# BowieHsu/tensorflow_ocr

Measured on AMD Instinct MI355X. Metric: images/sec training, 512x512 ICDAR, VGG-16 EAST, batch 32, 1/2/4/8 GPU, higher is better.
Workload: dtype f16; 1 GPU; VGG-16 model_vgg + dice loss train step, 512x512, batch 32 per GPU, f16 storage / f32 accumulate, Adam+EMA; global_batch=32, parallelism=dp1

## Files before the change

include/ocr_hip.h:

```cpp
#ifndef OCR_HIP_H_
#define OCR_HIP_H_

#include <stddef.h>
#include <stdint.h>

#ifdef __cplusplus
extern "C" {
#endif

#define OCR_ABI_VERSION 7

enum {
  OCR_OK = 0,
  OCR_ERR_INVALID_ARG = -1,
  OCR_ERR_UNSUPPORTED = -2,
  OCR_ERR_HIP = -3,
  OCR_ERR_WORKSPACE = -4,
  OCR_ERR_RCCL = -5
};

int ocr_abi_version(void);
const char* ocr_status_string(int status);
const char* ocr_storage_dtype(void);
uint32_t ocr_crc32c(const void* data, size_t n, uint32_t seed);
// ... 96 lines not shown
                        const void* bias, int flags, void* y, void* stats, void* stream);
size_t ocr_conv2d_stem_wgrad_workspace(int n, int h, int w, int cout);
int ocr_conv2d_stem_wgrad_f16(int n, int h, int w, int cout, const void* x4, const void* dy,
                              void* dw_hwio_f32, void* workspace, size_t ws_bytes, void* stream);
int ocr_conv2d_stem_wgrad_bn_f16(int n, int h, int w, int cout, const void* x4, const void* da, const void* bn_y,
                                 const void* bn_shift, const void* coef_a, const void* coef_b, const void* coef_c,
                                 int relu, void* dw, void* workspace, size_t ws_bytes, void* stream);
int ocr_pack_weights_f16(const void* w_hwio_f32, int taps, int cin, int cout, void* w_kc,
                         void* w_ck, void* stream);
int ocr_pack_weights_first_f16(const void* w_hwio_f32, int cout, void* w_first, void* stream);
size_t ocr_conv2d_first_moments_workspace(void);
int ocr_conv2d_first_moments_f16(int n, int h, int w, int cout, const void* x4, const void* w_first, void* stats_row,
                                 void* workspace, size_t ws_bytes, void* stream);
int ocr_conv2d_first_moments_keep_f16(int n, int h, int w, int cout, const void* x4, const void* w_first,
                                      void* stats_row, void* moments_f64, void* workspace, size_t ws_bytes, void* stream);
size_t ocr_pack_weights_batch_table_bytes(int n);
int ocr_pack_weights_batch_table(int n, const void* const* w_hwio_f32, const int* taps, const int* cin,
                                 const int* cout, void* const* w_kc, void* const* w_ck, const int* ld_ck,
                                 void* table_host, int* grid_out);
int ocr_pack_weights_batch_f16(const void* table_dev, int n, int grid, void* stream);
int ocr_pack_weights_small_f16(const void* w_f32, int cin, int cout, void* w_kc32, void* w_ck32,
                               void* stream);

int ocr_prep_images_f16(const void* images_f32, int64_t npix, float m0, float m1, float m2,
                        void* out_f16x4, void* stream);
int ocr_prep_images_norm_f16(const void* images_f32, int64_t npix, float m0, float m1, float m2,
                             float div, void* out_f16x4, void* stream);

size_t ocr_bn_reduce_workspace(int T, int C);
int ocr_bn_finalize(const void* partial, int T, int C, double count, const void* gamma,
// ... 448 lines not shown
```

tensorflow_ocr_amd/csrc/bn_pool.hip:

```cpp
#include "common.h"
#include "pool_gather.h"

namespace {

__global__ void prep_images_kernel(const float* __restrict__ img, half_t* __restrict__ out,
                                   size_t npix, float m0, float m1, float m2, float div) {
  size_t i = (size_t)blockIdx.x * blockDim.x + threadIdx.x;
  if (i >= npix) return;
  float r = (img[i * 3 + 0] - m0) / div, g = (img[i * 3 + 1] - m1) / div, b = (img[i * 3 + 2] - m2) / div;
  half4_t o = {(half_t)r, (half_t)g, (half_t)b, (half_t)0.f};
  *reinterpret_cast<half4_t*>(out + i * 4) = o;
}

struct BnFin {
  double count;
  const float *gamma, *beta;
  float eps, decay;
  float *moving_mean, *moving_var, *scale, *shift, *save_mean, *save_invstd;
};
struct BnBwdFin {
  float *dgamma, *dbeta;
};
struct BnBwdFinC {
  float *dgamma, *dbeta;
  const float *scale, *mean, *invstd;
  float inv_count;
  float *A, *B, *C;
};

constexpr int kTicketGroup = 32, kTicketGroups = 128;
__device__ unsigned ocr_bn_tickets[16 * 32 * (1 + kTicketGroups)];

template <typename FIN>
__device__ __forceinline__ void bn_fin_apply(const FIN& f, int c, double s, double q);

template <>
__device__ __forceinline__ void bn_fin_apply<BnFin>(const BnFin& f, int c, double s, double q) {
  double mean = s / f.count;
  double var = q / f.count - mean * mean;
  if (var < 0.0) var = 0.0;
  float invstd = (float)(1.0 / sqrt(var + (double)f.eps));
  float g = f.gamma ? f.gamma[c] : 1.f;
  float b = f.beta ? f.beta[c] : 0.f;
  float sc = g * invstd;
  f.scale[c] = sc;
  f.shift[c] = b - (float)mean * sc;
  if (f.save_mean) f.save_mean[c] = (float)mean;
  if (f.save_invstd) f.save_invstd[c] = invstd;
  if (f.moving_mean) {
    double unbiased = f.count > 1.0 ? var * f.count / (f.count - 1.0) : var;
    f.moving_mean[c] = f.moving_mean[c] * f.decay + (float)mean * (1.f - f.decay);
    f.moving_var[c] = f.moving_var[c] * f.decay + (float)unbiased * (1.f - f.decay);
  }
}

template <>
__device__ __forceinline__ void bn_fin_apply<BnBwdFin>(const BnBwdFin& f, int c, double s, double q) {
  f.dbeta[c] = (float)s;
  f.dgamma[c] = (float)q;
}

template <>
__device__ __forceinline__ void bn_fin_apply<BnBwdFinC>(const BnBwdFinC& f, int c, double s, double q) {
  f.dbeta[c] = (float)s;
  f.dgamma[c] = (float)q;
  const float sc = f.scale[c], mu = f.mean[c], is = f.invstd[c];
  const float k_dz = (float)s * f.inv_count, k_dzx = (float)q * f.inv_count;
  f.A[c] = sc;
  f.B[c] = -sc * is * k_dzx;
  f.C[c] = sc * (mu * is * k_dzx - k_dz);
}

static inline int red_rows(int T) {
  if (T <= 1024) return (T + 63) / 64 * 64;
  int rows = ((T + 15) / 16 + 31) / 32 * 32;
  if (rows < 256) rows = 256;
  if (rows > 2048) rows = 2048;
  return rows;
}

template <typename FIN>
__global__ __launch_bounds__(256) void reduce_finalize_kernel(const float* __restrict__ partial,
                                                              double* __restrict__ stage, int T, int C, int slot,
                                                              int rows, FIN fin) {
  __shared__ double red[16][2][64];
  __shared__ unsigned s_ticket;
  const int cl = threadIdx.x & 15, rl = threadIdx.x >> 4;
  const int c4 = blockIdx.y * 64 + cl * 4;
  const int t0 = blockIdx.x * rows;
  const int R = gridDim.x;
  double s[4] = {0.0, 0.0, 0.0, 0.0}, q[4] = {0.0, 0.0, 0.0, 0.0};
  const bool live = c4 < C;
  const bool vec = (C & 3) == 0;
  if (live) {
// ... 1489 lines not shown
```

tensorflow_ocr_amd/csrc/conv_first.hip:

```cpp
#include "common.h"
#include "conv_epilogue.h"

namespace {

constexpr int HW = 36;

struct FirstP {
  int n, h, w, cout, tiles_x, tiles_y, m_tiles, flags;
};

__device__ __forceinline__ void load_halo4(const half_t* __restrict__ x4, char* halo, int img, int h,
                                           int w, int iy0, int ix0) {
  for (int i = threadIdx.x; i < 10 * HW; i += 256) {
    const int hy = i / HW, hx = i - hy * HW;
    const int iy = iy0 + hy, ix = ix0 + hx;
    u32x2 v = {0u, 0u};
    if (iy >= 0 && iy < h && ix >= 0 && ix < w)
      v = *reinterpret_cast<const u32x2*>(x4 + (((size_t)img * h + iy) * w + ix) * 4);
    *reinterpret_cast<u32x2*>(halo + i * 8) = v;
  }
}

__device__ __forceinline__ void first_weights(const half_t* __restrict__ wf, int cout, int co0, int lane,
                                              half8_t (&a)[3][2]) {
// ... 365 lines not shown
        s2 += wv[i] * t;
      }
    }
    part[0][rl][threadIdx.x & 63] = s1;
    part[1][rl][threadIdx.x & 63] = s2;
    __syncthreads();
    if (threadIdx.x < 128) {
      const int k = threadIdx.x >> 6, cc = threadIdx.x & 63;
      if (c0 + cc < cout)
        row[k * cout + c0 + cc] = (float)(((part[k][0][cc] + part[k][1][cc]) + part[k][2][cc]) + part[k][3][cc]);
    }
    __syncthreads();
  }
}

__global__ __launch_bounds__(256) void first_wgrad_sums_kernel(const float* __restrict__ s1, int blocks,
                                                               const double* __restrict__ M,
                                                               const half_t* __restrict__ wf,
                                                               const float* __restrict__ A, const float* __restrict__ B,
                                                               const float* __restrict__ C, float* __restrict__ dw) {
  __shared__ double red[2][4][64];
  __shared__ double Mrow[32];
  const int k = blockIdx.x;
  const int ky = k / 9, kx = (k / 3) % 3, ch = k % 3;
  const int slot = ky * 10 + kx * 3 + ch;
  const int c = threadIdx.x & 63, bl = threadIdx.x >> 6;
  if (threadIdx.x < 32) Mrow[threadIdx.x] = M[k * 32 + threadIdx.x];
  float wj[7];
#pragma unroll
  for (int u = 0; u < 7; ++u) {
// ... 13 lines not shown
    for (int u = 0; u < 16; ++u) acc += (double)v[u];
  }
  __syncthreads();
  double mw = 0.0;
#pragma unroll
  for (int u = 0; u < 7; ++u) {
    const int j = bl + 4 * u;
    if (j < 27) mw += Mrow[j] * (double)wj[u];
  }
  red[0][bl][c] = acc;
  red[1][bl][c] = mw;
  __syncthreads();
  if (threadIdx.x < 64) {
    const double S1 = (red[0][0][c] + red[0][1][c]) + (red[0][2][c] + red[0][3][c]);
    const double MW = (red[1][0][c] + red[1][1][c]) + (red[1][2][c] + red[1][3][c]);
    dw[k * 64 + c] = (float)((double)A[c] * S1 + (double)B[c] * MW + (double)C[c] * M[27 * 32 + k]);
  }
}

__global__ void first_reduce_kernel(const float* __restrict__ partial, float* __restrict__ dw,
                                    int elems, int blocks) {
  int i = blockIdx.x * blockDim.x + threadIdx.x;
  if (i >= elems) return;
  float a = 0.f;
  for (int b = 0; b < blocks; ++b) a += partial[(size_t)b * elems + i];
  dw[i] = a;
}

__global__ void pack_first_kernel(const float* __restrict__ w, half_t* __restrict__ out, int cout) {
  int i = blockIdx.x * blockDim.x + threadIdx.x;
  if (i >= 3 * cout * 16) return;
// ... 142 lines not shown
                     cout, static_cast<float*>(stats_row), static_cast<double*>(moments_f64));
  return ocr_launch_status();
}

extern "C" int ocr_conv2d_first_wgrad_sums_f32(const void* s1_blocks, int blocks, const void* moments_f64,
                                               const void* w_first, int cout, const void* coef_a, const void* coef_b,
                                               const void* coef_c, void* dw, void* stream) {
  OCR_CHECK_ARG(s1_blocks && blocks > 0 && moments_f64 && w_first && coef_a && coef_b && coef_c && dw);
  OCR_CHECK_SHAPE(cout == 64);
  hipLaunchKernelGGL(first_wgrad_sums_kernel, dim3(27), dim3(256), 0, static_cast<hipStream_t>(stream),
                     static_cast<const float*>(s1_blocks), blocks, static_cast<const double*>(moments_f64),
                     static_cast<const half_t*>(w_first), static_cast<const float*>(coef_a),
                     static_cast<const float*>(coef_b), static_cast<const float*>(coef_c), static_cast<float*>(dw));
  return ocr_launch_status();
}
```

tensorflow_ocr_amd/graph.py:

```python
import contextlib
import math

import numpy as np
import torch

from . import _lib as L
from . import ops

F16, F32 = (torch.bfloat16 if L.STORAGE == "bf16" else torch.float16), torch.float32


class Variable:

    def __init__(self, name, shape, init, trainable, regularized):
        self.name = name
        self.shape = tuple(int(s) for s in shape)
        self.init = init
        self.trainable = trainable
        self.regularized = regularized
        self.data = None
        self.grad = None
        self.packed = {}

    @property
# ... 96 lines not shown
        for n, arr in sd.items():
            if n not in self.vars:
                if strict:
                    raise KeyError(n)
                continue
            v = self.vars[n]
            a = np.asarray(arr, dtype=np.float32).reshape(v.shape)
            v.data.copy_(torch.from_numpy(a))
        self.version += 1


class Act:

    __slots__ = ("_data", "grad", "requires_grad", "name", "bn_ctx", "bn_partial", "tail_ctx", "tail_partial",
                 "pending", "sub_grad", "deferred", "tail_fwd", "pending_owner", "consumed", "bn_fwd", "bias_ctx",
                 "bias_partial", "sole_consumer", "bias_done", "pool_grad", "takes_pool_grad", "first_s1")

    def __init__(self, data, requires_grad=True, name=""):
        self._data = data
        self.grad = None
        self.requires_grad = requires_grad
        self.name = name
        self.bn_ctx = None
        self.bn_partial = None
        self.tail_ctx = None
        self.tail_partial = None
        self.pending = None
        self.pending_owner = None
        self.consumed = False
        self.sub_grad = None
        self.deferred = None
        self.bias_ctx = None
        self.bias_partial = None
        self.bias_done = False
        self.sole_consumer = False
        self.takes_pool_grad = False
        self.pool_grad = None
        self.first_s1 = None
        self.bn_fwd = None
        self.tail_fwd = None

    @property
    def data(self):
        if self.deferred is not None:
            fill, self.deferred = self.deferred, None
            fill()
        return self._data

    @data.setter
    def data(self, value):
        self._data = value

    @property
# ... 281 lines not shown
```

tensorflow_ocr_amd/layers.py:

```python
import torch

from . import ops
from .graph import Act, F16, F32, constant, variance_scaling, xavier_uniform
from ._lib import CONV_ACCUM_F16, CONV_BIAS, CONV_RELU, CONV_STATS

BN_DECAY = 0.997
BN_EPS = 1e-5
FUSE_BN_REDUCE = __import__("os").environ.get("OCR_FUSE_BN", "1") == "1"


def _bn_vars(g, C):
    with g.variable_scope("BatchNorm"):
        gamma = g.get_variable("gamma", (C,), constant(1.0))
        beta = g.get_variable("beta", (C,), constant(0.0))
        mm = g.get_variable("moving_mean", (C,), constant(0.0), trainable=False)
        mv = g.get_variable("moving_variance", (C,), constant(1.0), trainable=False)
    return gamma, beta, mm, mv


def _packs(g, w, first):
    kh, kw, cin, cout = w.shape
    if first:
        def mk(old):
            t = old if old is not None else g.empty((3, cout, 16))
            ops.pack_weights_first(w.data, t)
            return t
        return g.packed(w, "first", mk), None

    def mk(old):
        if old is None:
            old = (g.empty((kh * kw, cout, cin)), g.empty((kh * kw, cin, cout)))
        ops.pack_weights(w.data, old[0], old[1])
        return old
    return g.packed(w, "kc_ck", mk)


FUSE_BIAS_POOL = __import__("os").environ.get("OCR_FUSE_BIAS_POOL", "1") == "1"
FUSE_BIAS_RELU = __import__("os").environ.get("OCR_FUSE_BIAS_RELU", "1") == "1"


# ... 2 lines not shown
    t = cache.get((n, value))
    if t is None:
        t = cache[(n, value)] = torch.full((n,), float(value), dtype=F32, device=g.device)
    return t


FUSE_BN_W4_MAXHW = int(__import__("os").environ.get("OCR_FUSE_BN_W4_MAXHW", "1000000"))
FUSE_BN_POOL_REDUCE = __import__("os").environ.get("OCR_FUSE_BN_POOL_REDUCE", "1") == "1"
FIRST_RECOMPUTE = __import__("os").environ.get("OCR_FIRST_RECOMPUTE", "1") == "1"
FIRST_DROP_Y = __import__("os").environ.get("OCR_FIRST_DROP_Y", "1") == "1"
FIRST_MOMENTS = __import__("os").environ.get("OCR_FIRST_MOMENTS", "1") == "1"
FIRST_WGRAD_RECOMPUTE = __import__("os").environ.get("OCR_FIRST_WGRAD_RECOMPUTE", "0") == "1"
GUEST_REDUCE = __import__("os").environ.get("OCR_GUEST_REDUCE", "1") == "1"
FUSE_FIRST_WGRAD = __import__("os").environ.get("OCR_FUSE_FIRST_WGRAD", "1") == "1"
FIRST_WGRAD_SUMS = __import__("os").environ.get("OCR_FIRST_WGRAD_SUMS", "1") == "1"


def conv2d(g, x, cout, k, scope, *, stride=1, rate=1, normalizer="bn", relu=True, pool=0,
           keep_full=True, is_training=True, bn_training=None, first=False, weight_decay=True,
           initializer=None):
    if g.precision == "f32":
        from . import layers_f32
        return layers_f32.conv2d(g, x, cout, k, scope, stride=stride, rate=rate, normalizer=normalizer,
                                 relu=relu, pool=pool, keep_full=keep_full, is_training=is_training,
                                 bn_training=bn_training, first=first, weight_decay=weight_decay,
                                 initializer=initializer)
    n, h, w, cin_x = x.shape
    cin = 3 if first else cin_x
    bn_training = is_training if bn_training is None else bn_training
    with g.variable_scope(scope):
        init = initializer or variance_scaling(g.rng)
        wv = g.get_variable("weights", (k, k, cin, cout), init, regularized=weight_decay)
        if normalizer == "bn":
            gamma, beta, mm, mv = _bn_vars(g, cout)
            bias = None
        else:
            bias = g.get_variable("biases", (cout,), constant(0.0))
    ws = g.workspace()
    w_fwd, w_dg = _packs(g, wv, first)
    if first:
        d = None
        oh, ow = h, w
        mt = ops.conv2d_first_num_mtiles(n, h, w)
    else:
        d = ops.conv_desc((n, h, w, cin), cout, k, k, stride, rate)
        oh, ow = d.oh, d.ow
        mt = ops.conv2d_num_mtiles(d)
    drop_y = (first and normalizer == "bn" and not pool and cout == 64 and FIRST_RECOMPUTE and FIRST_DROP_Y
              and (is_training if bn_training is None else bn_training) and FUSE_FIRST_WGRAD)
    y = ops.LazyFirstY(g.empty, x.data, w_fwd, (n, oh, ow, cout)) if drop_y else g.empty((n, oh, ow, cout))

    if normalizer == "bn":
        train_stats = bn_training
        flags = CONV_STATS if train_stats else 0
        part, stage = g.ws_small.two(mt * 2 * cout * 4, ops.bn_reduce_workspace(mt, cout))
        mt_fin = mt
        if first and drop_y and train_stats and FIRST_MOMENTS:
            if FIRST_WGRAD_SUMS:
                y.moments = g.empty((32 * 32,), torch.float64)
            ops.conv2d_first_moments(x.data, w_fwd, part, cout, ws, moments=y.moments)
            mt_fin = 1
        elif first:
            ops.conv2d_first(x.data, w_fwd, None if drop_y else y, flags, None, part if train_stats else None, cout=cout)
        else:
            d.flags = flags
            ops.conv2d(d, x.data, w_fwd, y, None, part if train_stats else None)
        scale, shift = g.empty((cout,), F32), g.empty((cout,), F32)
        mean, invstd = g.empty((cout,), F32), g.empty((cout,), F32)
        if train_stats:
            ops.bn_finalize(part, mt_fin, cout, float(n) * oh * ow, gamma.data, beta.data, BN_EPS, BN_DECAY,
                            mm.data, mv.data, scale, shift, mean, invstd, stage)
        else:
            ops.bn_inference_params(gamma.data, beta.data, mm.data, mv.data, BN_EPS, scale, shift)
        full = pooled = None
        argmax = y_pool = argmax_full = None
        if pool:
            pooled = g.empty((n, (oh + 1) // 2, (ow + 1) // 2, cout))
            if keep_full:
                full = g.empty((n, oh, ow, cout))
                if train_stats and relu and ops.guest_apply_ok((n, oh, ow, cout)) and oh % 2 == 0 and ow % 2 == 0:
                    argmax_full = g.empty(pooled.shape, torch.uint8)
                    ops.bn_relu_pool_idx(y, scale, shift, relu, full, pooled, argmax_full, None)
                else:
                    ops.bn_relu(y, scale, shift, relu, 2, full, pooled)
# ... 10 lines not shown
        a_full = Act(full, name=scope) if full is not None else None
        a_pool = Act(pooled, name=scope + "/pool") if pooled is not None else None
        if not pool and train_stats:
            a_full.bn_ctx = (y, scale, shift, mean, invstd, relu)
        if pool and argmax is not None and y_pool is not None:
            a_pool.bn_ctx = (y_pool, scale, shift, mean, invstd, relu)

        def backward():
            if not train_stats:
                raise NotImplementedError("backward through inference-mode batch norm")
            da_full = a_full.grad if a_full is not None else None
            da_pool = a_pool.grad if a_pool is not None else None
            if first and a_full is not None and a_full.first_s1 is not None:
                part_f, T_f = a_full.bn_partial
                coef = (g.empty((cout,), F32), g.empty((cout,), F32), g.empty((cout,), F32))
                ops.bn_bwd_coefficients(part_f, T_f, cout, float(n) * oh * ow, scale, mean, invstd, gamma.grad,
                                        beta.grad, coef, ws)
                ops.conv2d_first_wgrad_sums(a_full.first_s1, y.moments, w_fwd, coef, wv.grad)
                a_full.bn_partial = None
                a_full.first_s1 = None
                return
            if da_full is None and da_pool is None:
                return
            if pool and da_pool is None:
                da_pool = g.empty(a_pool.data.shape)
                ops.fill_(da_pool, 0.0)
            if not pool and da_full is None:
                return
            if first and not pool and a_full.bn_partial is not None and FUSE_FIRST_WGRAD:
                part_f, T_f = a_full.bn_partial
                coef = (g.empty((cout,), F32), g.empty((cout,), F32), g.empty((cout,), F32))
                ops.bn_bwd_coefficients(part_f, T_f, cout, float(n) * oh * ow, scale, mean, invstd, gamma.grad,
                                        beta.grad, coef, ws)
# ... 225 lines not shown
        out.grad = None
    g.record(backward)
    return out


def prep_images(g, images, means=(123.68, 116.78, 103.94), div=1.0):
    if images.shape[-1] != len(means):
        raise ValueError("len(means) must match the number of channels")
    if g.precision == "f32":
        from . import layers_f32
        if div != 1.0:
            raise NotImplementedError("input normalisation is folded into the f16 path only")
        return layers_f32.prep_images(g, images, means)
    n, h, w, _ = images.shape
    x4 = g.empty((n, h, w, 4))
    ops.prep_images(images, x4, means, div)
    return Act(x4, requires_grad=False, name="images")


class SmallAct:
    __slots__ = ("data", "grad")

    def __init__(self, data):
        self.data = data
        self.grad = None


def head_conv_bn(g, feat, names, couts, is_training=True, relu=True):
    n, h, w, cin = feat.shape
    C = sum(couts)
    ws, ws_small = g.workspace(), g.ws_small
    with g.variable_scope("+".join(names)):
# ... 362 lines not shown
```

tensorflow_ocr_amd/ops.py:

```python
import ctypes
from ctypes import byref, c_double, c_float, c_int, c_int64, c_size_t

import torch

from . import _lib as L
from ._lib import ConvDesc, CONV_ACCUM_F16, CONV_BIAS, CONV_RELU, CONV_STATS, ptr

F16, F32 = (torch.bfloat16 if L.STORAGE == "bf16" else torch.float16), torch.float32


def _st():
    return L.stream_ptr()


def same_pad(size, k, stride, dilation=1):
    k_eff = (k - 1) * dilation + 1
    out = -(-size // stride)
    total = max((out - 1) * stride + k_eff - size, 0)
    return out, total // 2


class Workspace:

    def __init__(self, device, nbytes=64 << 20):
# ... 287 lines not shown


def conv2d_first(x4, w_first, y, flags=0, bias=None, stats=None, cout=None):
    n, h, w, _ = x4.shape
    cout = y.shape[-1] if y is not None else cout
    L.call("ocr_conv2d_first_f16", c_int(n), c_int(h), c_int(w), c_int(cout), ptr(x4), ptr(w_first),
           ptr(bias), c_int(flags), ptr(y), ptr(stats), _st())


def conv2d_first_moments(x4, w_first, row, cout, ws, moments=None):
    n, h, w, _ = x4.shape
    nbytes = L.call_size("ocr_conv2d_first_moments_workspace")
    buf = ws.get(nbytes)
    L.call("ocr_conv2d_first_moments_keep_f16", c_int(n), c_int(h), c_int(w), c_int(cout), ptr(x4), ptr(w_first),
           ptr(row), ptr(moments), ptr(buf), c_size_t(nbytes), _st())


def conv2d_first_wgrad(x4, dy, dw, ws):
    n, h, w, _ = x4.shape
    cout = dy.shape[-1]
    nbytes = L.call_size("ocr_conv2d_first_wgrad_workspace", c_int(n), c_int(h), c_int(w), c_int(cout))
    buf = ws.get(nbytes)
    L.call("ocr_conv2d_first_wgrad_f16", c_int(n), c_int(h), c_int(w), c_int(cout), ptr(x4), ptr(dy),
           ptr(dw), ptr(buf), c_size_t(nbytes), _st())


def conv2d_first_wgrad_bn(x4, da, y, shift, coef, relu, dw, ws, w_first=None):
    n, h, w, _ = x4.shape
    cout = da.shape[-1]
    nbytes = L.call_size("ocr_conv2d_first_wgrad_workspace", c_int(n), c_int(h), c_int(w), c_int(cout))
# ... 1001 lines not shown
```

Before: 1814 images/sec.

## Fuse image prep into first-conv moments and merge first-layer BN finalize/tail kernels

Image normalisation is deferred and folded into a new first-layer front kernel that reads the raw f32 images, writes the f16 padded input and accumulates the input moment matrix in one pass. A finish kernel then reduces the moments, packs the first-layer weights and applies the BN finalize. A tail kernel merges the backward BN coefficients with the first-layer weight gradient. Together these remove a separate prep pass and several small launches, at the cost of more complex kernels with ticket-based last-block reductions.

```diff
diff --git a/include/ocr_hip.h b/include/ocr_hip.h
--- a/include/ocr_hip.h
+++ b/include/ocr_hip.h
@@ -134,6 +134,18 @@
                                  void* workspace, size_t ws_bytes, void* stream);
 int ocr_conv2d_first_moments_keep_f16(int n, int h, int w, int cout, const void* x4, const void* w_first,
                                       void* stats_row, void* moments_f64, void* workspace, size_t ws_bytes, void* stream);
+int ocr_conv2d_first_front_f16(int n, int h, int w, const void* images_f32, float m0, float m1, float m2, float div,
+                               void* x4, void* workspace, size_t ws_bytes, void* stream);
+int ocr_conv2d_first_finish_f16(int n, int h, int w, int cout, const void* w_hwio_f32, void* w_first, void* stats_row,
+                                void* moments_f64, const void* gamma, const void* beta, float eps, float decay,
+                                void* moving_mean, void* moving_var, void* scale, void* shift, void* save_mean,
+                                void* save_invstd, void* workspace, size_t ws_bytes, void* stream);
+size_t ocr_conv2d_first_tail_workspace(int T);
+int ocr_conv2d_first_tail_f32(const void* partial, int T, double count, const void* scale, const void* save_mean,
+                              const void* save_invstd, void* dgamma, void* dbeta, void* coef_a, void* coef_b,
+                              void* coef_c, const void* s1_blocks, int blocks, const void* moments_f64,
+                              const void* w_first, int cout, void* dw_hwio_f32, void* workspace, size_t ws_bytes,
+                              void* stream);
 size_t ocr_pack_weights_batch_table_bytes(int n);
 int ocr_pack_weights_batch_table(int n, const void* const* w_hwio_f32, const int* taps, const int* cin,
                                  const int* cout, void* const* w_kc, void* const* w_ck, const int* ld_ck,
diff --git a/tensorflow_ocr_amd/csrc/bn_fin.h b/tensorflow_ocr_amd/csrc/bn_fin.h
--- /dev/null
+++ b/tensorflow_ocr_amd/csrc/bn_fin.h
@@ -0,0 +1,73 @@
+#pragma once
+#include "common.h"
+
+namespace {
+
+struct BnFin {
+  double count;
+  const float *gamma, *beta;
+  float eps, decay;
+  float *moving_mean, *moving_var, *scale, *shift, *save_mean, *save_invstd;
+};
+struct BnBwdFin {
+  float *dgamma, *dbeta;
+};
+struct BnBwdFinC {
+  float *dgamma, *dbeta;
+  const float *scale, *mean, *invstd;
+  float inv_count;
+  float *A, *B, *C;
+};
+
+template <typename FIN>
+__device__ __forceinline__ void bn_fin_apply(const FIN& f, int c, double s, double q);
+
+template <>
+__device__ __forceinline__ void bn_fin_apply<BnFin>(const BnFin& f, int c, double s, double q) {
+  double mean = s / f.count;
+  double var = q / f.count - mean * mean;
+  if (var < 0.0) var = 0.0;
+  float invstd = (float)(1.0 / sqrt(var + (double)f.eps));
+  float g = f.gamma ? f.gamma[c] : 1.f;
+  float b = f.beta ? f.beta[c] : 0.f;
+  float sc = g * invstd;
+  f.scale[c] = sc;
+  f.shift[c] = b - (float)mean * sc;
+  if (f.save_mean) f.save_mean[c] = (float)mean;
+  if (f.save_invstd) f.save_invstd[c] = invstd;
+  if (f.moving_mean) {
+    double unbiased = f.count > 1.0 ? var * f.count / (f.count - 1.0) : var;
+    const float keep = 1.f - f.decay;
+    float mm_old = f.moving_mean[c] * f.decay, mm_new = (float)mean * keep;
+    asm volatile("" : "+v"(mm_old), "+v"(mm_new));
+    f.moving_mean[c] = mm_old + mm_new;
+    f.moving_var[c] = __builtin_fmaf(keep, (float)unbiased, f.moving_var[c] * f.decay);
+  }
+}
+
+template <>
+__device__ __forceinline__ void bn_fin_apply<BnBwdFin>(const BnBwdFin& f, int c, double s, double q) {
+  f.dbeta[c] = (float)s;
+  f.dgamma[c] = (float)q;
+}
+
+template <>
+__device__ __forceinline__ void bn_fin_apply<BnBwdFinC>(const BnBwdFinC& f, int c, double s, double q) {
+  f.dbeta[c] = (float)s;
+  f.dgamma[c] = (float)q;
+  const float sc = f.scale[c], mu = f.mean[c], is = f.invstd[c];
+  const float k_dz = (float)s * f.inv_count, k_dzx = (float)q * f.inv_count;
+  f.A[c] = sc;
+  f.B[c] = -sc * is * k_dzx;
+  f.C[c] = sc * (mu * is * k_dzx - k_dz);
+}
+
+static inline int red_rows(int T) {
+  if (T <= 1024) return (T + 63) / 64 * 64;
+  int rows = ((T + 15) / 16 + 31) / 32 * 32;
+  if (rows < 256) rows = 256;
+  if (rows > 2048) rows = 2048;
+  return rows;
+}
+
+}
diff --git a/tensorflow_ocr_amd/csrc/bn_pool.hip b/tensorflow_ocr_amd/csrc/bn_pool.hip
--- a/tensorflow_ocr_amd/csrc/bn_pool.hip
+++ b/tensorflow_ocr_amd/csrc/bn_pool.hip
@@ -1,4 +1,5 @@
 #include "common.h"
+#include "bn_fin.h"
 #include "pool_gather.h"
 
 namespace {
@@ -12,72 +13,9 @@
   *reinterpret_cast<half4_t*>(out + i * 4) = o;
 }
 
-struct BnFin {
-  double count;
-  const float *gamma, *beta;
-  float eps, decay;
-  float *moving_mean, *moving_var, *scale, *shift, *save_mean, *save_invstd;
-};
-struct BnBwdFin {
-  float *dgamma, *dbeta;
-};
-struct BnBwdFinC {
-  float *dgamma, *dbeta;
-  const float *scale, *mean, *invstd;
-  float inv_count;
-  float *A, *B, *C;
-};
 
 constexpr int kTicketGroup = 32, kTicketGroups = 128;
 __device__ unsigned ocr_bn_tickets[16 * 32 * (1 + kTicketGroups)];
-
-template <typename FIN>
-__device__ __forceinline__ void bn_fin_apply(const FIN& f, int c, double s, double q);
-
-template <>
-__device__ __forceinline__ void bn_fin_apply<BnFin>(const BnFin& f, int c, double s, double q) {
-  double mean = s / f.count;
-  double var = q / f.count - mean * mean;
-  if (var < 0.0) var = 0.0;
-  float invstd = (float)(1.0 / sqrt(var + (double)f.eps));
-  float g = f.gamma ? f.gamma[c] : 1.f;
-  float b = f.beta ? f.beta[c] : 0.f;
-  float sc = g * invstd;
-  f.scale[c] = sc;
-  f.shift[c] = b - (float)mean * sc;
-  if (f.save_mean) f.save_mean[c] = (float)mean;
-  if (f.save_invstd) f.save_invstd[c] = invstd;
-  if (f.moving_mean) {
-    double unbiased = f.count > 1.0 ? var * f.count / (f.count - 1.0) : var;
-    f.moving_mean[c] = f.moving_mean[c] * f.decay + (float)mean * (1.f - f.decay);
-    f.moving_var[c] = f.moving_var[c] * f.decay + (float)unbiased * (1.f - f.decay);
-  }
-}
-
-template <>
-__device__ __forceinline__ void bn_fin_apply<BnBwdFin>(const BnBwdFin& f, int c, double s, double q) {
-  f.dbeta[c] = (float)s;
-  f.dgamma[c] = (float)q;
-}
-
-template <>
-__device__ __forceinline__ void bn_fin_apply<BnBwdFinC>(const BnBwdFinC& f, int c, double s, double q) {
-  f.dbeta[c] = (float)s;
-  f.dgamma[c] = (float)q;
-  const float sc = f.scale[c], mu = f.mean[c], is = f.invstd[c];
-  const float k_dz = (float)s * f.inv_count, k_dzx = (float)q * f.inv_count;
-  f.A[c] = sc;
-  f.B[c] = -sc * is * k_dzx;
-  f.C[c] = sc * (mu * is * k_dzx - k_dz);
-}
-
-static inline int red_rows(int T) {
-  if (T <= 1024) return (T + 63) / 64 * 64;
-  int rows = ((T + 15) / 16 + 31) / 32 * 32;
-  if (rows < 256) rows = 256;
-  if (rows > 2048) rows = 2048;
-  return rows;
-}
 
 template <typename FIN>
 __global__ __launch_bounds__(256) void reduce_finalize_kernel(const float* __restrict__ partial,
diff --git a/tensorflow_ocr_amd/csrc/conv_first.hip b/tensorflow_ocr_amd/csrc/conv_first.hip
--- a/tensorflow_ocr_amd/csrc/conv_first.hip
+++ b/tensorflow_ocr_amd/csrc/conv_first.hip
@@ -1,4 +1,5 @@
 #include "common.h"
+#include "bn_fin.h"
 #include "conv_epilogue.h"
 
 namespace {
@@ -403,6 +404,10 @@
   }
 }
 
+__device__ __forceinline__ float first_dw_value(float A, float B, float C, double S1, double MW, double m) {
+  return (float)__builtin_fma(m, (double)C, __builtin_fma(S1, (double)A, MW * (double)B));
+}
+
 __global__ __launch_bounds__(256) void first_wgrad_sums_kernel(const float* __restrict__ s1, int blocks,
                                                                const double* __restrict__ M,
                                                                const half_t* __restrict__ wf,
@@ -446,7 +451,355 @@
   if (threadIdx.x < 64) {
     const double S1 = (red[0][0][c] + red[0][1][c]) + (red[0][2][c] + red[0][3][c]);
     const double MW = (red[1][0][c] + red[1][1][c]) + (red[1][2][c] + red[1][3][c]);
-    dw[k * 64 + c] = (float)((double)A[c] * S1 + (double)B[c] * MW + (double)C[c] * M[27 * 32 + k]);
+    dw[k * 64 + c] = first_dw_value(A[c], B[c], C[c], S1, MW, M[27 * 32 + k]);
+  }
+}
+
+constexpr int FHW = 34;
+struct FrontPrep {
+  float m0, m1, m2, div;
+};
+
+__global__ __launch_bounds__(256) void first_front_kernel(FirstP p, const float* __restrict__ img, FrontPrep pr,
+                                                          half_t* __restrict__ x4, float* __restrict__ slab) {
+  __shared__ __attribute__((aligned(16))) char halo[10 * HW * 8];
+  __shared__ __attribute__((aligned(16))) char patch[256 * PSTRF];
+  __shared__ float red[4][1024];
+  const int tid = threadIdx.x, lane = tid & 63, wave = tid >> 6;
+  const int li = lane & 15, g = lane >> 4;
+  const int q = li >> 2, pp = li & 3, hh = g >> 1, gc = g & 1;
+  const int a_lane = (8 * hh + q) * PSTRF + (16 * gc + 4 * pp) * 2;
+  f32x16 acc;
+#pragma unroll
+  for (int e = 0; e < 16; ++e) acc[e] = 0.f;
+  int hy[2], hx[2];
+#pragma unroll
+  for (int j = 0; j < 2; ++j) {
+    const int i = tid + 256 * j;
+    hy[j] = i / FHW;
+    hx[j] = i - hy[j] * FHW;
+  }
+  float raw[2][3];
+  auto fetch = [&](int mt) {
+    const int txi = mt % p.tiles_x;
+    const int tmp = mt / p.tiles_x;
+    const int tyi = tmp % p.tiles_y;
+    const int im = tmp / p.tiles_y;
+#pragma unroll
+    for (int j = 0; j < 2; ++j) {
+      const int iy = tyi * TILE_H - 1 + hy[j], ix = txi * TILE_W - 1 + hx[j];
+      raw[j][0] = raw[j][1] = raw[j][2] = 0.f;
+      if (hy[j] < 10 && iy >= 0 && iy < p.h && ix >= 0 && ix < p.w) {
+        const float* s = img + (((size_t)im * p.h + iy) * p.w + ix) * 3;
+        raw[j][0] = s[0]; raw[j][1] = s[1]; raw[j][2] = s[2];
+      }
+    }
+  };
+  if ((int)blockIdx.x < p.m_tiles) fetch(blockIdx.x);
+  for (int mt = blockIdx.x; mt < p.m_tiles; mt += gridDim.x) {
+    const int txi = mt % p.tiles_x;
+    const int tmp = mt / p.tiles_x;
+    const int tyi = tmp % p.tiles_y;
+    const int im = tmp / p.tiles_y;
+    __syncthreads();
+#pragma unroll
+    for (int j = 0; j < 2; ++j) {
+      if (hy[j] < 10) {
+        const int iy = tyi * TILE_H - 1 + hy[j], ix = txi * TILE_W - 1 + hx[j];
+        const bool in_image = iy >= 0 && iy < p.h && ix >= 0 && ix < p.w;
+        half4_t o = {(half_t)0.f, (half_t)0.f, (half_t)0.f, (half_t)0.f};
+        if (in_image) {
+          const float r = (raw[j][0] - pr.m0) / pr.div, gr = (raw[j][1] - pr.m1) / pr.div, b = (raw[j][2] - pr.m2) / pr.div;
+          o = half4_t{(half_t)r, (half_t)gr, (half_t)b, (half_t)0.f};
+          if (hy[j] >= 1 && hy[j] <= TILE_H && hx[j] >= 1 && hx[j] <= TILE_W)
+            *reinterpret_cast<half4_t*>(x4 + (((size_t)im * p.h + iy) * p.w + ix) * 4) = o;
+        }
+        *reinterpret_cast<half4_t*>(halo + (hy[j] * HW + hx[j]) * 8) = o;
+      }
+    }
+    if (mt + (int)gridDim.x < p.m_tiles) fetch(mt + gridDim.x);
+    __syncthreads();
+    {
+      const int ty = tid >> 5, tx = tid & 31;
+      const bool inside = tyi * TILE_H + ty < p.h && txi * TILE_W + tx < p.w;
+      half_t row[32];
+#pragma unroll
+      for (int k = 27; k < 32; ++k) row[k] = (half_t)0.f;
+      row[27] = inside ? (half_t)1.f : (half_t)0.f;
+#pragma unroll
+      for (int ky = 0; ky < 3; ++ky)
+#pragma unroll
+        for (int kx = 0; kx < 3; ++kx) {
+          half4_t xv = *reinterpret_cast<const half4_t*>(halo + ((ty + ky) * HW + tx + kx) * 8);
+#pragma unroll
+          for (int c = 0; c < 3; ++c) row[(ky * 3 + kx) * 3 + c] = inside ? xv[c] : (half_t)0.f;
+        }
+#pragma unroll
+      for (int k = 0; k < 4; ++k) {
+        half8_t v;
+#pragma unroll
+        for (int e = 0; e < 8; ++e) v[e] = row[k * 8 + e];
+        *reinterpret_cast<half8_t*>(patch + tid * PSTRF + k * 16) = v;
+      }
+    }
+    __syncthreads();
+#pragma unroll
+    for (int s = 0; s < 4; ++s) {
+      const int k0 = (wave * 4 + s) * 16;
+      half8_t a = tr_pair_f(patch + a_lane + k0 * PSTRF, 4 * PSTRF);
+      acc = OCR_MFMA_32x32x16(a, a, acc, 0, 0, 0);
+    }
+  }
+  const int r = lane & 31, h2 = lane >> 5;
+#pragma unroll
+  for (int e = 0; e < 16; ++e) red[wave][((e & 3) + 8 * (e >> 2) + 4 * h2) * 32 + r] = acc[e];
+  __syncthreads();
+  for (int i = tid; i < 1024; i += 256)
+    slab[(size_t)blockIdx.x * 1024 + i] = (red[0][i] + red[1][i]) + (red[2][i] + red[3][i]);
+}
+
+__device__ unsigned ocr_first_tickets[2];
+__device__ __forceinline__ void put_f64(double* p, double v) {
+  __hip_atomic_store(reinterpret_cast<unsigned long long*>(p), __builtin_bit_cast(unsigned long long, v), __ATOMIC_RELAXED,
+                     __HIP_MEMORY_SCOPE_AGENT);
+}
+__device__ __forceinline__ unsigned long long get_u64(const double* p) {
+  return __hip_atomic_load(reinterpret_cast<const unsigned long long*>(p), __ATOMIC_RELAXED, __HIP_MEMORY_SCOPE_AGENT);
+}
+__device__ __forceinline__ bool last_arriver(unsigned* ticket, unsigned total, unsigned* s_flag) {
+  asm volatile("s_waitcnt vmcnt(0)" ::: "memory");
+  __syncthreads();
+  if (threadIdx.x == 0) {
+    const unsigned last = __hip_atomic_fetch_add(ticket, 1u, __ATOMIC_RELAXED, __HIP_MEMORY_SCOPE_AGENT) == total - 1u;
+    if (last) __hip_atomic_store(ticket, 0u, __ATOMIC_RELAXED, __HIP_MEMORY_SCOPE_AGENT);
+    *s_flag = last;
+  }
+  __syncthreads();
+  return *s_flag != 0u;
+}
+
+struct FinishP {
+  const float* slab;
+  int blocks;
+  double* stage;
+  const float* w;
+  half_t* wf;
+  int cout;
+  float* row;
+  double* m_out;
+  BnFin fin;
+};
+__global__ __launch_bounds__(256) void first_finish_kernel(FinishP f) {
+  __shared__ double M[32 * 32];
+  __shared__ double part[2][4][64];
+  __shared__ float rowf[2][64];
+  __shared__ unsigned s_last;
+  const int tid = threadIdx.x;
+  {
+    const int per = (f.blocks + 31) / 32;
+    const int b0 = blockIdx.x * per, b1 = b0 + per < f.blocks ? b0 + per : f.blocks;
+    const int col = blockIdx.y * 256 + tid;
+    double a = 0.0;
+    for (int b = b0; b < b1; b += 16) {
+      float v[16];
+#pragma unroll
+      for (int u = 0; u < 16; ++u) v[u] = b + u < b1 ? f.slab[(size_t)(b + u) * 1024 + col] : 0.f;
+#pragma unroll
+      for (int u = 0; u < 16; ++u) a += (double)v[u];
+    }
+    put_f64(f.stage + (size_t)blockIdx.x * 1024 + col, a);
+  }
+  if (!last_arriver(&ocr_first_tickets[0], gridDim.x * gridDim.y, &s_last)) return;
+  for (int i = tid; i < 1024; i += 256) {
+    double a = 0.0;
+#pragma unroll
+    for (int b0 = 0; b0 < 32; b0 += 16) {
+      unsigned long long u[16];
+#pragma unroll
+      for (int k = 0; k < 16; ++k) u[k] = get_u64(f.stage + (size_t)(b0 + k) * 1024 + i);
+#pragma unroll
+      for (int k = 0; k < 16; ++k) a += __builtin_bit_cast(double, u[k]);
+    }
+    M[i] = a;
+    if (f.m_out != nullptr) f.m_out[i] = a;
+  }
+  const int cout = f.cout;
+  for (int i = tid; i < 3 * cout * 16; i += 256) {
+    const int k = i & 15, co = (i >> 4) % cout, ky = (i >> 4) / cout;
+    const int kx = k >> 2, c = k & 3;
+    const float v = (kx < 3 && c < 3) ? f.w[((ky * 3 + kx) * 3 + c) * cout + co] : 0.f;
+    f.wf[i] = (half_t)v;
+  }
+  __syncthreads();
+  for (int c0 = 0; c0 < cout; c0 += 64) {
+    const int co = c0 + (tid & 63), rl = tid >> 6;
+    double s1 = 0.0, s2 = 0.0;
+    if (co < cout) {
+      double wv[27];
+#pragma unroll
+      for (int k = 0; k < 27; ++k) wv[k] = (double)(float)(half_t)f.w[k * cout + co];
+      for (int i = rl; i < 27; i += 4) {
+        const double wi = (double)(float)(half_t)f.w[i * cout + co];
+        s1 += wi * M[27 * 32 + i];
+        double t = 0.0;
+#pragma unroll
+        for (int j = 0; j < 27; ++j) t += M[i * 32 + j] * wv[j];
+        s2 += wi * t;
+      }
+    }
+    part[0][rl][tid & 63] = s1;
+    part[1][rl][tid & 63] = s2;
+    __syncthreads();
+    if (tid < 128) {
+      const int k = tid >> 6, cc = tid & 63;
+      if (c0 + cc < cout) {
+        const float v = (float)(((part[k][0][cc] + part[k][1][cc]) + part[k][2][cc]) + part[k][3][cc]);
+        f.row[k * cout + c0 + cc] = v;
+        rowf[k][cc] = v;
+      }
+    }
+    __syncthreads();
+    if (tid < 64 && c0 + tid < cout) {
+      double s = 0.0, q = 0.0;
+      s += (double)rowf[0][tid];
+      q += (double)rowf[1][tid];
+      bn_fin_apply<BnFin>(f.fin, c0 + tid, s, q);
+    }
+  }
+}
+
+struct TailP {
+  const float* partial;
+  int T, rows, R;
+  double* stage;
+  double* sums;
+  const float* s1;
+  int blocks;
+  const double* M;
+  const half_t* wf;
+  float* dw;
+  BnBwdFinC fin;
+};
+__global__ __launch_bounds__(256) void first_tail_kernel(TailP f) {
+  __shared__ double red[16][2][64];
+  __shared__ double Mrow[32];
+  __shared__ float coef[3][64];
+  __shared__ unsigned s_last;
+  const int tid = threadIdx.x;
+  if ((int)blockIdx.x < f.R) {
+    const int cl = tid & 15, rl = tid >> 4;
+    const int c4 = cl * 4;
+    const int t0 = blockIdx.x * f.rows;
+    const int t1 = min(t0 + f.rows, f.T);
+    double s[4] = {0.0, 0.0, 0.0, 0.0}, q[4] = {0.0, 0.0, 0.0, 0.0};
+    for (int t = t0 + rl; t < t1; t += 64) {
+      f32x4 a[4], b[4];
+#pragma unroll
+      for (int k = 0; k < 4; ++k) {
+        const int tt = t + 16 * k;
+        a[k] = f32x4{0.f, 0.f, 0.f, 0.f};
+        b[k] = f32x4{0.f, 0.f, 0.f, 0.f};
+        if (tt < t1) {
+          a[k] = *reinterpret_cast<const f32x4*>(f.partial + ((size_t)tt * 2 + 0) * 64 + c4);
+          b[k] = *reinterpret_cast<const f32x4*>(f.partial + ((size_t)tt * 2 + 1) * 64 + c4);
+        }
+      }
+#pragma unroll
+      for (int k = 0; k < 4; ++k)
+#pragma unroll
+        for (int e = 0; e < 4; ++e) {
+          s[e] += (double)a[k][e];
+          q[e] += (double)b[k][e];
+        }
+    }
+#pragma unroll
+    for (int e = 0; e < 4; ++e) {
+      red[rl][0][cl * 4 + e] = s[e];
+      red[rl][1][cl * 4 + e] = q[e];
+    }
+    __syncthreads();
+    const int which = tid >> 6;
+    if (which < 2) {
+      double tot = 0.0;
+#pragma unroll
+      for (int k = 0; k < 16; ++k) tot += red[k][which][tid & 63];
+      put_f64(f.stage + ((size_t)blockIdx.x * 2 + which) * 64 + (tid & 63), tot);
+    }
+  } else {
+    const int k = blockIdx.x - f.R;
+    const int ky = k / 9, kx = (k / 3) % 3, ch = k % 3;
+    const int slot = ky * 10 + kx * 3 + ch;
+    const int c = tid & 63, bl = tid >> 6;
+    if (tid < 32) Mrow[tid] = f.M[k * 32 + tid];
+    float wj[7];
+#pragma unroll
+    for (int u = 0; u < 7; ++u) {
+      const int j = bl + 4 * u;
+      const int jy = j / 9, jx = (j / 3) % 3, jc = j % 3;
+      wj[u] = j < 27 ? (float)f.wf[((size_t)(jy * 64 + c)) * 16 + jx * 4 + jc] : 0.f;
+    }
+    double acc = 0.0;
+    for (int b0 = bl; b0 < f.blocks; b0 += 64) {
+      float v[16];
+#pragma unroll
+      for (int u = 0; u < 16; ++u) {
+        const int b = b0 + 4 * u;
+        v[u] = b < f.blocks ? f.s1[((size_t)b * 32 + slot) * 64 + c] : 0.f;
+      }
+#pragma unroll
+      for (int u = 0; u < 16; ++u) acc += (double)v[u];
+    }
+    __syncthreads();
+    double mw = 0.0;
+#pragma unroll
+    for (int u = 0; u < 7; ++u) {
+      const int j = bl + 4 * u;
+      if (j < 27) mw += Mrow[j] * (double)wj[u];
+    }
+    double* lanes = &red[0][0][0];
+    lanes[tid] = acc;
+    lanes[256 + tid] = mw;
+    __syncthreads();
+    if (tid < 64) {
+      const double S1 = (lanes[c] + lanes[64 + c]) + (lanes[128 + c] + lanes[192 + c]);
+      const double MW = (lanes[256 + c] + lanes[320 + c]) + (lanes[384 + c] + lanes[448 + c]);
+      put_f64(f.sums + ((size_t)k * 2 + 0) * 64 + c, S1);
+      put_f64(f.sums + ((size_t)k * 2 + 1) * 64 + c, MW);
+    }
+  }
+  if (!last_arriver(&ocr_first_tickets[1], gridDim.x, &s_last)) return;
+  const int R = f.R;
+  if (R == 1) {
+    if (tid < 128) red[0][tid >> 6][tid & 63] = __builtin_bit_cast(double, get_u64(f.stage + tid));
+  } else {
+    const int col = tid & 127, lane2 = tid >> 7;
+    double acc = 0.0;
+    for (int r0 = lane2; r0 < R; r0 += 16) {
+      unsigned long long u[8];
+#pragma unroll
+      for (int k = 0; k < 8; ++k) {
+        const int r = r0 + 2 * k;
+        u[k] = r < R ? get_u64(f.stage + ((size_t)r * 2 + (col >> 6)) * 64 + (col & 63)) : 0ull;
+      }
+#pragma unroll
+      for (int k = 0; k < 8; ++k) acc += __builtin_bit_cast(double, u[k]);
+    }
+    red[lane2][col >> 6][col & 63] = acc;
+  }
+  __syncthreads();
+  if (tid < 64) {
+    if (R == 1) bn_fin_apply<BnBwdFinC>(f.fin, tid, red[0][0][tid], red[0][1][tid]);
+    else bn_fin_apply<BnBwdFinC>(f.fin, tid, red[0][0][tid] + red[1][0][tid], red[0][1][tid] + red[1][1][tid]);
+    coef[0][tid] = f.fin.A[tid];
+    coef[1][tid] = f.fin.B[tid];
+    coef[2][tid] = f.fin.C[tid];
+  }
+  __syncthreads();
+  for (int i = tid; i < 27 * 64; i += 256) {
+    const int k = i >> 6, c = i & 63;
+    const double S1 = __builtin_bit_cast(double, get_u64(f.sums + ((size_t)k * 2 + 0) * 64 + c));
+    const double MW = __builtin_bit_cast(double, get_u64(f.sums + ((size_t)k * 2 + 1) * 64 + c));
+    f.dw[i] = first_dw_value(coef[0][c], coef[1][c], coef[2][c], S1, MW, f.M[27 * 32 + k]);
   }
 }
 
@@ -619,3 +972,79 @@
                      static_cast<const float*>(coef_b), static_cast<const float*>(coef_c), static_cast<float*>(dw));
   return ocr_launch_status();
 }
+
+extern "C" int ocr_conv2d_first_front_f16(int n, int h, int w, const void* images_f32, float m0, float m1, float m2,
+                                          float div, void* x4, void* workspace, size_t ws_bytes, void* stream) {
+  FirstP p;
+  int rc = fill(&p, n, h, w, 64, 0);
+  if (rc != OCR_OK) return rc;
+  OCR_CHECK_ARG(images_f32 && x4 && workspace && div != 0.f);
+  OCR_CHECK_ARG(((uintptr_t)x4 & 7) == 0 && ((uintptr_t)images_f32 & 3) == 0);
+  if (ws_bytes < ocr_conv2d_first_moments_workspace() || ((uintptr_t)workspace & 7)) return OCR_ERR_WORKSPACE;
+  const int blocks = p.m_tiles < FM_WGS ? p.m_tiles : FM_WGS;
+  hipLaunchKernelGGL(first_front_kernel, dim3(blocks), dim3(256), 0, static_cast<hipStream_t>(stream), p,
+                     static_cast<const float*>(images_f32), FrontPrep{m0, m1, m2, div}, static_cast<half_t*>(x4),
+                     static_cast<float*>(workspace));
+  return ocr_launch_status();
+}
+
+extern "C" int ocr_conv2d_first_finish_f16(int n, int h, int w, int cout, const void* w_hwio_f32, void* w_first,
+                                           void* stats_row, void* moments_f64, const void* gamma, const void* beta,
+                                           float eps, float decay, void* moving_mean, void* moving_var, void* scale,
+                                           void* shift, void* save_mean, void* save_invstd, void* workspace,
+                                           size_t ws_bytes, void* stream) {
+  FirstP p;
+  int rc = fill(&p, n, h, w, cout, 0);
+  if (rc != OCR_OK) return rc;
+  OCR_CHECK_ARG(w_hwio_f32 && w_first && stats_row && scale && shift && workspace);
+  OCR_CHECK_ARG((moving_mean == nullptr) == (moving_var == nullptr));
+  OCR_CHECK_ARG(((uintptr_t)moments_f64 & 7) == 0);
+  if (ws_bytes < ocr_conv2d_first_moments_workspace() || ((uintptr_t)workspace & 7)) return OCR_ERR_WORKSPACE;
+  const int blocks = p.m_tiles < FM_WGS ? p.m_tiles : FM_WGS;
+  FinishP f;
+  f.slab = static_cast<const float*>(workspace);
+  f.blocks = blocks;
+  f.stage = reinterpret_cast<double*>(static_cast<char*>(workspace) + (size_t)FM_WGS * 1024 * sizeof(float));
+  f.w = static_cast<const float*>(w_hwio_f32);
+  f.wf = static_cast<half_t*>(w_first);
+  f.cout = cout;
+  f.row = static_cast<float*>(stats_row);
+  f.m_out = static_cast<double*>(moments_f64);
+  f.fin = BnFin{(double)n * h * w, static_cast<const float*>(gamma), static_cast<const float*>(beta), eps, decay,
+                static_cast<float*>(moving_mean), static_cast<float*>(moving_var), static_cast<float*>(scale),
+                static_cast<float*>(shift), static_cast<float*>(save_mean), static_cast<float*>(save_invstd)};
+  hipLaunchKernelGGL(first_finish_kernel, dim3(32, 4), dim3(256), 0, static_cast<hipStream_t>(stream), f);
+  return ocr_launch_status();
+}
+
+extern "C" size_t ocr_conv2d_first_tail_workspace(int T) {
+  if (T <= 0) return 0;
+  return ((size_t)ocr_cdiv(T, red_rows(T)) + 27) * 2 * 64 * sizeof(double);
+}
+extern "C" int ocr_conv2d_first_tail_f32(const void* partial, int T, double count, const void* scale,
+                                         const void* save_mean, const void* save_invstd, void* dgamma, void* dbeta,
+                                         void* coef_a, void* coef_b, void* coef_c, const void* s1_blocks, int blocks,
+                                         const void* moments_f64, const void* w_first, int cout, void* dw,
+                                         void* workspace, size_t ws_bytes, void* stream) {
+  OCR_CHECK_ARG(partial && scale && save_mean && save_invstd && dgamma && dbeta && coef_a && coef_b && coef_c);
+  OCR_CHECK_ARG(s1_blocks && blocks > 0 && moments_f64 && w_first && dw && workspace && T > 0 && count > 0);
+  OCR_CHECK_SHAPE(cout == 64);
+  if (ws_bytes < ocr_conv2d_first_tail_workspace(T) || ((uintptr_t)workspace & 7)) return OCR_ERR_WORKSPACE;
+  TailP f;
+  f.partial = static_cast<const float*>(partial);
+  f.T = T;
+  f.rows = red_rows(T);
+  f.R = ocr_cdiv(T, f.rows);
+  f.stage = static_cast<double*>(workspace);
+  f.sums = f.stage + (size_t)f.R * 2 * 64;
+  f.s1 = static_cast<const float*>(s1_blocks);
+  f.blocks = blocks;
+  f.M = static_cast<const double*>(moments_f64);
+  f.wf = static_cast<const half_t*>(w_first);
+  f.dw = static_cast<float*>(dw);
+  f.fin = BnBwdFinC{static_cast<float*>(dgamma), static_cast<float*>(dbeta), static_cast<const float*>(scale),
+                    static_cast<const float*>(save_mean), static_cast<const float*>(save_invstd), (float)(1.0 / count),
+                    static_cast<float*>(coef_a), static_cast<float*>(coef_b), static_cast<float*>(coef_c)};
+  hipLaunchKernelGGL(first_tail_kernel, dim3(f.R + 27), dim3(256), 0, static_cast<hipStream_t>(stream), f);
+  return ocr_launch_status();
+}
diff --git a/tensorflow_ocr_amd/graph.py b/tensorflow_ocr_amd/graph.py
--- a/tensorflow_ocr_amd/graph.py
+++ b/tensorflow_ocr_amd/graph.py
@@ -134,7 +134,7 @@
 
     __slots__ = ("_data", "grad", "requires_grad", "name", "bn_ctx", "bn_partial", "tail_ctx", "tail_partial",
                  "pending", "sub_grad", "deferred", "tail_fwd", "pending_owner", "consumed", "bn_fwd", "bias_ctx",
-                 "bias_partial", "sole_consumer", "bias_done", "pool_grad", "takes_pool_grad", "first_s1")
+                 "bias_partial", "sole_consumer", "bias_done", "pool_grad", "takes_pool_grad", "first_s1", "front_src")
 
     def __init__(self, data, requires_grad=True, name=""):
         self._data = data
@@ -157,6 +157,7 @@
         self.takes_pool_grad = False
         self.pool_grad = None
         self.first_s1 = None
+        self.front_src = None
         self.bn_fwd = None
         self.tail_fwd = None
 
diff --git a/tensorflow_ocr_amd/layers.py b/tensorflow_ocr_amd/layers.py
--- a/tensorflow_ocr_amd/layers.py
+++ b/tensorflow_ocr_amd/layers.py
@@ -2,7 +2,7 @@
 
 from . import ops
 from .graph import Act, F16, F32, constant, variance_scaling, xavier_uniform
-from ._lib import CONV_ACCUM_F16, CONV_BIAS, CONV_RELU, CONV_STATS
+from ._lib import CONV_ACCUM_F16, CONV_BIAS, CONV_RELU, CONV_STATS, STORAGE
 
 BN_DECAY = 0.997
 BN_EPS = 1e-5
@@ -18,12 +18,13 @@
     return gamma, beta, mm, mv
 
 
-def _packs(g, w, first):
+def _packs(g, w, first, defer=False):
     kh, kw, cin, cout = w.shape
     if first:
         def mk(old):
             t = old if old is not None else g.empty((3, cout, 16))
-            ops.pack_weights_first(w.data, t)
+            if not defer:
+                ops.pack_weights_first(w.data, t)
             return t
         return g.packed(w, "first", mk), None
 
@@ -56,6 +57,7 @@
 GUEST_REDUCE = __import__("os").environ.get("OCR_GUEST_REDUCE", "1") == "1"
 FUSE_FIRST_WGRAD = __import__("os").environ.get("OCR_FUSE_FIRST_WGRAD", "1") == "1"
 FIRST_WGRAD_SUMS = __import__("os").environ.get("OCR_FIRST_WGRAD_SUMS", "1") == "1"
+FIRST_FRONT = __import__("os").environ.get("OCR_FIRST_FRONT", "1") == "1"
 
 
 def conv2d(g, x, cout, k, scope, *, stride=1, rate=1, normalizer="bn", relu=True, pool=0,
@@ -79,7 +81,13 @@
         else:
             bias = g.get_variable("biases", (cout,), constant(0.0))
     ws = g.workspace()
-    w_fwd, w_dg = _packs(g, wv, first)
+    drop_y = (first and normalizer == "bn" and not pool and cout == 64 and FIRST_RECOMPUTE and FIRST_DROP_Y
+              and (is_training if bn_training is None else bn_training) and FUSE_FIRST_WGRAD)
+    front = None
+    if (drop_y and FIRST_MOMENTS and FIRST_FRONT and STORAGE == "f16" and k == 3 and x.deferred is not None
+            and x.front_src is not None):
+        front, x.front_src, x.deferred = x.front_src, None, None
+    w_fwd, w_dg = _packs(g, wv, first, defer=front is not None)
     if first:
         d = None
         oh, ow = h, w
@@ -88,8 +96,6 @@
         d = ops.conv_desc((n, h, w, cin), cout, k, k, stride, rate)
         oh, ow = d.oh, d.ow
         mt = ops.conv2d_num_mtiles(d)
-    drop_y = (first and normalizer == "bn" and not pool and cout == 64 and FIRST_RECOMPUTE and FIRST_DROP_Y
-              and (is_training if bn_training is None else bn_training) and FUSE_FIRST_WGRAD)
     y = ops.LazyFirstY(g.empty, x.data, w_fwd, (n, oh, ow, cout)) if drop_y else g.empty((n, oh, ow, cout))
 
     if normalizer == "bn":
@@ -97,7 +103,15 @@
         flags = CONV_STATS if train_stats else 0
         part, stage = g.ws_small.two(mt * 2 * cout * 4, ops.bn_reduce_workspace(mt, cout))
         mt_fin = mt
-        if first and drop_y and train_stats and FIRST_MOMENTS:
+        scale, shift = g.empty((cout,), F32), g.empty((cout,), F32)
+        mean, invstd = g.empty((cout,), F32), g.empty((cout,), F32)
+        if front is not None:
+            if FIRST_WGRAD_SUMS:
+                y.moments = g.empty((32 * 32,), torch.float64)
+            images, means, div = front
+            ops.conv2d_first_front(images, means, div, x.data, wv.data, w_fwd, part, y.moments,
+                                   (gamma.data, beta.data, BN_EPS, BN_DECAY, mm.data, mv.data, scale, shift, mean, invstd), ws)
+        elif first and drop_y and train_stats and FIRST_MOMENTS:
             if FIRST_WGRAD_SUMS:
                 y.moments = g.empty((32 * 32,), torch.float64)
             ops.conv2d_first_moments(x.data, w_fwd, part, cout, ws, moments=y.moments)
@@ -107,9 +121,9 @@
         else:
             d.flags = flags
             ops.conv2d(d, x.data, w_fwd, y, None, part if train_stats else None)
-        scale, shift = g.empty((cout,), F32), g.empty((cout,), F32)
-        mean, invstd = g.empty((cout,), F32), g.empty((cout,), F32)
-        if train_stats:
+        if front is not None:
+            pass
+        elif train_stats:
             ops.bn_finalize(part, mt_fin, cout, float(n) * oh * ow, gamma.data, beta.data, BN_EPS, BN_DECAY,
                             mm.data, mv.data, scale, shift, mean, invstd, stage)
         else:
@@ -150,9 +164,13 @@
             if first and a_full is not None and a_full.first_s1 is not None:
                 part_f, T_f = a_full.bn_partial
                 coef = (g.empty((cout,), F32), g.empty((cout,), F32), g.empty((cout,), F32))
-                ops.bn_bwd_coefficients(part_f, T_f, cout, float(n) * oh * ow, scale, mean, invstd, gamma.grad,
-                                        beta.grad, coef, ws)
-                ops.conv2d_first_wgrad_sums(a_full.first_s1, y.moments, w_fwd, coef, wv.grad)
+                if FIRST_FRONT and STORAGE == "f16":
+                    ops.conv2d_first_tail(part_f, T_f, float(n) * oh * ow, scale, mean, invstd, gamma.grad, beta.grad, coef,
+                                          a_full.first_s1, y.moments, w_fwd, wv.grad, ws)
+                else:
+                    ops.bn_bwd_coefficients(part_f, T_f, cout, float(n) * oh * ow, scale, mean, invstd, gamma.grad,
+                                            beta.grad, coef, ws)
+                    ops.conv2d_first_wgrad_sums(a_full.first_s1, y.moments, w_fwd, coef, wv.grad)
                 a_full.bn_partial = None
                 a_full.first_s1 = None
                 return
@@ -408,8 +426,16 @@
         return layers_f32.prep_images(g, images, means)
     n, h, w, _ = images.shape
     x4 = g.empty((n, h, w, 4))
-    ops.prep_images(images, x4, means, div)
-    return Act(x4, requires_grad=False, name="images")
+    act = Act(x4, requires_grad=False, name="images")
+    if FIRST_FRONT and STORAGE == "f16" and images.dtype == F32 and images.is_contiguous():
+        def fill():
+            act.front_src = None
+            ops.prep_images(images, x4, means, div)
+        act.front_src = (images, tuple(means), div)
+        act.deferred = fill
+    else:
+        ops.prep_images(images, x4, means, div)
+    return act
 
 
 class SmallAct:
diff --git a/tensorflow_ocr_amd/ops.py b/tensorflow_ocr_amd/ops.py
--- a/tensorflow_ocr_amd/ops.py
+++ b/tensorflow_ocr_amd/ops.py
@@ -325,6 +325,28 @@
     buf = ws.get(nbytes)
     L.call("ocr_conv2d_first_moments_keep_f16", c_int(n), c_int(h), c_int(w), c_int(cout), ptr(x4), ptr(w_first),
            ptr(row), ptr(moments), ptr(buf), c_size_t(nbytes), _st())
+
+
+def conv2d_first_front(images, means, div, x4, w_hwio, w_first, row, moments, bn, ws):
+    n, h, w, _ = x4.shape
+    cout = w_hwio.shape[-1]
+    nbytes = L.call_size("ocr_conv2d_first_moments_workspace")
+    buf = ws.get(nbytes)
+    L.call("ocr_conv2d_first_front_f16", c_int(n), c_int(h), c_int(w), ptr(images), c_float(means[0]), c_float(means[1]),
+           c_float(means[2]), c_float(div), ptr(x4), ptr(buf), c_size_t(nbytes), _st())
+    gamma, beta, eps, decay, mm, mv, scale, shift, mean, invstd = bn
+    L.call("ocr_conv2d_first_finish_f16", c_int(n), c_int(h), c_int(w), c_int(cout), ptr(w_hwio), ptr(w_first), ptr(row),
+           ptr(moments), ptr(gamma), ptr(beta), c_float(eps), c_float(decay), ptr(mm), ptr(mv), ptr(scale), ptr(shift),
+           ptr(mean), ptr(invstd), ptr(buf), c_size_t(nbytes), _st())
+
+
+def conv2d_first_tail(partial, T, count, scale, save_mean, save_invstd, dgamma, dbeta, coef, s1, moments, w_first, dw, ws):
+    a, b, c = coef
+    nbytes = L.call_size("ocr_conv2d_first_tail_workspace", c_int(T))
+    buf = ws.get(nbytes)
+    L.call("ocr_conv2d_first_tail_f32", ptr(partial), c_int(T), c_double(count), ptr(scale), ptr(save_mean),
+           ptr(save_invstd), ptr(dgamma), ptr(dbeta), ptr(a), ptr(b), ptr(c), ptr(s1), c_int(s1.shape[0]), ptr(moments),
+           ptr(w_first), c_int(dw.shape[-1]), ptr(dw), ptr(buf), c_size_t(nbytes), _st())
 
 
 def conv2d_first_wgrad(x4, dy, dw, ws):
```

New measurement: 1814 images/sec. No clear change (-0.0%).
